# BolinLai/CSTS

Measured on AMD Instinct MI355X. Metric: clips/sec training (fwd+bwd) CSTS-Ego4D 16x256^2 bf16, higher is better.
Workload: dtype bf16; 1 GPU; CSTS_Ego4D_Gaze_Forecast.yaml train step (fwd + KLDiv + 0.05*EgoNCE + bwd + clip + AdamW), 16x256^2 video + 24 kHz STFT audio, b=4/GPU; mode=train, global_batch=4, frames=16, crop=256, parallelism=dp1, step=hip_graph, hip_graph=True, rccl_ranks=1

## Files before the change

csts_amd/csrc/gemm.hip:

```cpp
#include "common.h"
#include "gemm_shared.h"
#include <type_traits>
#include <cstdio>
#include <cstdlib>

namespace {

constexpr int BM = 128, BN = 128, BK = 32, NT_ = 256;
constexpr int KC_LD_BF = BK + 8;
constexpr int OC_LD_BF = 128 + 32;
constexpr int KC_LD_F = BK + 1;
constexpr int OC_LD_F = 128 + 4;

template <bool F32> struct Cmp;
template <> struct Cmp<false> { typedef bf16 T; };
template <> struct Cmp<true> { typedef float T; };


__device__ __forceinline__ void load8(const void* p, int dt, int64_t idx, int nvalid, bool vec, float (&o)[8]) {
  if (nvalid >= 8 && vec) {
    ld8_as_f32(p, dt, idx, o);
  } else {
#pragma unroll
    for (int j = 0; j < 8; ++j) o[j] = (j < nvalid) ? ld_as_f32(p, dt, idx + j) : 0.f;
// ... 1030 lines not shown
bool v3_ok(const csts_gemm_args* a, int split) {
  return v2_ok(a) && a->layout == CSTS_GEMM_NT && a->a_dt == CSTS_BF16 && a->b_dt == CSTS_BF16 && a->K % 16 == 0 &&
         split == 1 && a->colsum == nullptr &&
         a->M * a->lda < (int64_t(1) << 30) && a->N * a->ldb < (int64_t(1) << 30);
}
bool pick3(const csts_gemm_args* a, int split, int* mt, int* stages) {
  if (a->algo != 0 || a->tile_rows != 0 || !v3_ok(a, split) || a->M < 256 || a->res_up[3] > 0) return false;
  if (cdiv(a->M, 128) * cdiv(a->N, BN) >= 512 || a->K < 768) return false;
  *mt = 1;
  *stages = 3;
  return true;
}

bool pick4(const csts_gemm_args* a, int split, int* variant) {
  static const bool enabled = [] { const char* e = getenv("CSTS_GEMM4"); return !(e && e[0] == '0'); }();
  if (!enabled || a->algo != 0 || a->tile_rows != 0 || !v3_ok(a, split) || a->K % 64 != 0 || a->M < 2048 || a->res_up[3] > 0) return false;
  if (a->c_dt == CSTS_F32 && a->residual != nullptr) {
    static const bool res_on = [] { const char* e = getenv("CSTS_GEMM4_RES"); return !(e && e[0] == '0'); }();
    if (!res_on || a->r_dt != CSTS_F32 || a->res_row_mod != 0 || a->epilogue != CSTS_EPI_NONE || a->M % 128 != 0) return false;
    static const bool t64 = [] { const char* e = getenv("CSTS_GEMM4_T64"); return e && (e[0] == '1' || e[0] == '3'); }();
    if (t64 && a->N % 192 == 0 && a->M % 64 == 0 && a->K >= 384 && (a->M / 128) * (a->N / 192) <= 128 && (a->M / 64) * (a->N / 192) >= 64) {
      *variant = 73;
      return true;
    }
    if (a->N % 192 != 0 || (a->M / 128) * (a->N / 192) < 128) return false;
    *variant = 63;
    return true;
  }
  if (a->c_dt != CSTS_BF16 || a->residual != nullptr) return false;
  const int64_t rows = cdiv(a->M, 128);
  {
// ... 12 lines not shown
    return true;
  }
  const int64_t t128 = rows * cdiv(a->N, 128);
  if (a->N % 128 == 0 && t128 >= 128 && t128 <= 512) {
    *variant = a->K >= 1024 ? 33 : 32;
    return true;
  }
  return false;
}

bool pick5(const csts_gemm_args* a, int split) {
  static const bool enabled = [] { const char* e = getenv("CSTS_GEMM5"); return !(e && e[0] == '0'); }();
  if (!enabled || a->algo != 0 || a->tile_rows != 0 || a->M < 16384) return false;
  static const bool k384 = [] { const char* e = getenv("CSTS_GEMM5_K384"); return e && e[0] == '1'; }();
  if (a->K == 384 && !k384) return false;
  return csts_gemm5_ok(a, split);
}

template <int MT>
void launch3_mt(const Params& p, int stages, dim3 grid, hipStream_t s) {
  if (stages == 2) hipLaunchKernelGGL((gemm3_kernel<MT, 2>), grid, dim3(256), 0, s, p);
  else if (stages == 4 && MT < 4) hipLaunchKernelGGL((gemm3_kernel<MT, (MT < 4 ? 4 : 3)>), grid, dim3(256), 0, s, p);
  else hipLaunchKernelGGL((gemm3_kernel<MT, 3>), grid, dim3(256), 0, s, p);
}
void launch3(Params p, int mt, int stages, int wpc, hipStream_t s) {
  const int64_t ntiles = cdiv(p.M, 64 * mt) * p.ntiles_n;
  p.ntiles = ntiles;
  const int stage_bytes = (64 * mt + 128) * 128;
  const int fit = std::max(1, (160 * 1024) / (stages * stage_bytes));
  if (wpc <= 0 || wpc > fit) wpc = fit;
// ... 58 lines not shown
  else hipLaunchKernelGGL((gemm_tiny_kernel<LAYOUT, true>), dim3((unsigned)cdiv(outs, 4)), dim3(256), 0, s, p);
}


enum Family { TINY, GENERIC, V2, RING3, G4, G5 };
struct Route {
  Family family;
  int split;
  bool det;
  int tile_rows, stages;
  int variant, wpc;
  int64_t k_chunk;
  int nsplit;
};

int route(const csts_gemm_args* a, Route* r) {
  *r = Route{};
  r->split = r->nsplit = 1;
  if (tiny_ok(a)) {
    r->family = TINY;
    return 0;
  }
  const int split = r->split = a->split_k > 1 ? a->split_k : 1;
  r->det = split > 1 && a->workspace != nullptr;
  const bool use_v2 = v2_ok(a);
  const int bk = use_v2 ? BK2 : BK;
  r->k_chunk = cdiv(cdiv(a->K, bk), split) * bk;
  r->nsplit = (int)cdiv(a->K, r->k_chunk);
  const int forced = a->algo % 1000;
  if (a->res_up[3] > 0) {
    const int Ti = a->res_up[0], Hi = a->res_up[1], Wi = a->res_up[2], To = a->res_up[3], Ho = a->res_up[4], Wo = a->res_up[5];
    auto p2 = [](int v) { return v > 0 && (v & (v - 1)) == 0; };
    CSTS_REQUIRE(a->residual != nullptr && a->res_row_mod == 0 && split == 1, "res_up needs a residual, no res_row_mod, split_k == 1");
    CSTS_REQUIRE(Ti > 0 && Hi > 0 && Wi > 0 && p2(To) && p2(Ho) && p2(Wo), "res_up: fine grid sizes must be powers of two");
    CSTS_REQUIRE(To >= Ti && Ho >= Hi && Wo >= Wi && a->M % ((int64_t)To * Ho * Wo) == 0, "res_up: M must be B * To * Ho * Wo");
    CSTS_REQUIRE(forced < 300, "res_up is not available in the persistent LDS-DMA kernels");
  }
  if (forced >= 300 && forced < 400) {
    CSTS_REQUIRE(v3_ok(a, split), "algo 3xx (persistent LDS-DMA NT kernel) not applicable to this problem");
    const int code = forced - 300, mt = code / 10, st = code % 10;
    CSTS_REQUIRE((mt == 1 || mt == 2 || mt == 4) && st >= 2 && st <= 4 && !(mt == 4 && st == 4), "bad algo 3xx code");
    r->family = RING3; r->tile_rows = 64 * mt; r->stages = st; r->wpc = a->algo / 1000;
    return 0;
  }
  if (forced >= 400 && forced < 500) {
    CSTS_REQUIRE(v3_ok(a, split), "algo 4xx (8-wave LDS-DMA NT kernel) not applicable to this problem");
    CSTS_REQUIRE(a->K % 64 == 0, "algo 4xx needs K % 64 == 0 (no k-tail instantiations)");
    r->family = G4; r->variant = forced - 400; r->wpc = a->algo / 1000;
    return 0;
  }
  if (forced == 500 || forced == 503 || forced == 506) {
    CSTS_REQUIRE(csts_gemm5_ok(a, split), "algo 500 (streaming thin-operand NT kernel) not applicable to this problem");
    r->family = G5;
    return 0;
  }
  int mt3;
  if (pick5(a, split)) r->family = G5;
  else if (pick4(a, split, &r->variant)) r->family = G4;
  else if (pick3(a, split, &mt3, &r->stages)) { r->family = RING3; r->tile_rows = 64 * mt3; }
  else if (use_v2) { r->family = V2; r->tile_rows = pick_tile_rows(a, cdiv(a->N, BN) * r->nsplit); }
  else { r->family = GENERIC; r->tile_rows = BM; }
  return 0;
}

Params fill_params(const csts_gemm_args* a, const Route& r) {
  Params p{};
// ... 156 lines not shown
```

csts_amd/csrc/gemm4.hip:

```cpp
#include "gemm_shared.h"
#include <algorithm>
#include <cstdio>
#include <type_traits>

#ifdef CSTS_GEMM4_STAMPS
#define G4_STAMP() do { if (stamp_on && nstamp < 500) stamp_buf[nstamp++] = (unsigned long long)__builtin_amdgcn_s_memtime(); } while (0)
#else
#define G4_STAMP() do { } while (0)
#endif

namespace {

template <int WM, int MT, int NT, int S, int NP_ = 0> struct G4 {
  static constexpr int NP = NP_;
  static constexpr int DB = (MT * NT >= 6) ? 1 : 2;
  static constexpr int NWAVES = WM * 2, NTHR = 64 * (NWAVES + NP);
  static constexpr int DW = NP > 0 ? NP : NWAVES;
  static constexpr int BM = WM * 32 * MT, BN = 64 * NT;
  static constexpr int A_BYTES = BM * 128, B_BYTES = BN * 128, STAGE = A_BYTES + B_BYTES;
  static constexpr int NA = BM / 8 / DW, NB = BN / 8 / DW, LPT = NA + NB;
  static constexpr int FIT = (160 * 1024) / (S * STAGE);
  static constexpr int WG = NP > 0 ? 1 : (FIT < 1 ? 1 : (FIT > 2 ? 2 : FIT));
  static constexpr int WPS = (WG * (NWAVES + NP) + 3) / 4;
  static_assert(BM % (8 * DW) == 0 && BN % (8 * DW) == 0, "pieces must divide over the issuing waves");
// ... 108 lines not shown
  int cidx = 0, cstage = 0;

  for (int64_t t = t_first; t < t_end; t += stride) {
    f32x16 acc[MT][NT];
#pragma unroll
    for (int i = 0; i < MT; ++i)
#pragma unroll
      for (int j = 0; j < NT; ++j)
#pragma unroll
        for (int r = 0; r < 16; ++r) acc[i][j][r] = 0.f;
    const int64_t m0 = (t / p.ntiles_n) * BM + wm * 32 * MT + (lane & 31), n0 = (t % p.ntiles_n) * BN + wn * 32 * NT + 4 * hi;

    auto kstep = [&](auto nks_tag, int kt) {
      constexpr int NKS = decltype(nks_tag)::value;
      if constexpr (NP == 0) {
        constexpr int EPI_ST = (FORM == 0 || FORM == 5) ? 0 : MT * NT * 2;
        static_assert(2 * LPT + EPI_ST <= 63, "vmcnt immediate");
        const int ahead = min(S - 2, total_k - 1 - cidx);
        if (EPI_ST > 0 && STORE_AWARE && t != t_first && kt < S - 1) {
          if (S >= 4 && ahead == 2) wait_vm<2 * LPT + EPI_ST>();
          else if (S >= 3 && ahead >= 1) wait_vm<LPT + EPI_ST>();
          else wait_vm<EPI_ST>();
        } else {
          if (S >= 4 && ahead == 2) wait_vm<2 * LPT>();
          else if (S >= 3 && ahead >= 1) wait_vm<LPT>();
          else wait_vm<0>();
        }
      }
      G4_STAMP();
      __builtin_amdgcn_s_barrier();
      G4_STAMP();
// ... 18 lines not shown
      frags(0, 0);
#pragma unroll
      for (int ks = 0; ks < NKS; ++ks) {
        if (DB == 2 && ks + 1 < NKS) frags(ks + 1, (ks + 1) & 1);
        if (refill) {
#pragma unroll
          for (int i = 0; i < LPT; ++i) {
            const bool mine = (NKS == 4) ? (i * 4 / LPT == ks) : (ks == 0);
            if (mine) issue(i, st, k0, full);
          }
        }
#pragma unroll
        for (int i = 0; i < MT; ++i)
#pragma unroll
          for (int j = 0; j < NT; ++j)
            if constexpr (FORM == 5) acc[i][j] = CSTS_MFMA16(fa[ks & (DB - 1)][i], fb[ks & (DB - 1)][j], acc[i][j], 0, 0, 0);
            else acc[i][j] = CSTS_MFMA16(fb[ks & (DB - 1)][j], fa[ks & (DB - 1)][i], acc[i][j], 0, 0, 0);
        if (DB == 1 && ks + 1 < NKS) frags(ks + 1, 0);
      }
      if (refill) advance();
      G4_STAMP();
    };
    for (int kt = 0; kt < nk_full; ++kt) kstep(std::integral_constant<int, 4>(), kt);
    if constexpr (KTAIL) {
      if (k_tail == 1) kstep(std::integral_constant<int, 1>(), nk_full);
      else if (k_tail == 2) kstep(std::integral_constant<int, 2>(), nk_full);
      else if (k_tail == 3) kstep(std::integral_constant<int, 3>(), nk_full);
    }

    G4_STAMP();
    if constexpr (FORM == 5) {
      float* __restrict__ Cf = reinterpret_cast<float*>(p.C);
      const float* __restrict__ Rf = reinterpret_cast<const float*>(p.residual);
      const int64_t mb = m0 - (lane & 31) + 4 * hi, nb = n0 - 4 * hi + (lane & 31);
#pragma unroll
      for (int mi = 0; mi < MT; ++mi) {
        const int64_t mrow = mb + mi * 32;
        float sc[16];
        if (p.row_scale != nullptr) {
          const int64_t s_lo = (mrow - 4 * hi) / p.rows_per_scale, s_hi = (mrow - 4 * hi + 31) / p.rows_per_scale;
          if (s_lo == s_hi) {
            const float v = p.row_scale[s_lo];
#pragma unroll
            for (int r = 0; r < 16; ++r) sc[r] = v;
          } else {
#pragma unroll
            for (int r = 0; r < 16; ++r) sc[r] = p.row_scale[(mrow + (r & 3) + 8 * (r >> 2)) / p.rows_per_scale];
          }
        }
        float rr[2][16];
        const int64_t nwave = n0 - 4 * hi;
        auto loads = [&](int ni, int buf) {
          if (nwave + ni * 32 >= p.N) return;
#pragma unroll
          for (int r = 0; r < 16; ++r) rr[buf][r] = Rf[(mrow + (r & 3) + 8 * (r >> 2)) * p.ldr + nb + ni * 32];
        };
        loads(0, 0);
#pragma unroll
        for (int ni = 0; ni < NT; ++ni) {
          const int cur = ni & 1;
          if (nwave + ni * 32 >= p.N) break;
          const float bq = p.bias != nullptr ? p.bias[nb + ni * 32] : 0.f;
          if (ni + 1 < NT) loads(ni + 1, cur ^ 1);
#pragma unroll
          for (int r = 0; r < 16; ++r) {
            float v = acc[mi][ni][r] + bq;
            if (p.row_scale != nullptr) v *= sc[r];
            Cf[(mrow + (r & 3) + 8 * (r >> 2)) * p.ldc + nb + ni * 32] = v + rr[cur][r];
          }
          __builtin_amdgcn_sched_barrier(0);
        }
      }
    } else if constexpr (FORM != 0) {
      bf16* __restrict__ Cb = reinterpret_cast<bf16*>(p.C);
      bf16* __restrict__ Xb = reinterpret_cast<bf16*>(p.aux);
      const int hi16 = hi << 4;
      auto fwd = [&](auto gelu_tag) {
        constexpr bool GELU = decltype(gelu_tag)::value;
        const float* __restrict__ bias = p.bias;
#pragma unroll
        for (int mi = 0; mi < MT; ++mi) {
          const int64_t m = m0 + mi * 32;
          float bu[NT];
#pragma unroll
          for (int ni = 0; ni < NT; ++ni) bu[ni] = bias[n0 - 4 * hi + ni * 32 + (lane & 31)];
// ... 105 lines not shown
        }
        st4x4(p.C, p.c_dt, m * p.ldc + n0 + ni * 32, o, mok, n0 + ni * 32, p.N, hi);
      }
    }
    }
    G4_STAMP();
  }
  wait_vm<0>();
  G4_STAMP();
#ifdef CSTS_GEMM4_STAMPS
  if (stamp_on) { stamp_buf[0] = (unsigned long long)nstamp; stamp_buf[501] = (unsigned long long)__builtin_amdgcn_s_memrealtime(); }
#endif
}

int gemm4_form(const Params& p, int BM, int BN) {
  if (p.M % BM == 0 && p.N % 32 == 0 && p.c_dt == CSTS_F32 && p.residual != nullptr && p.r_dt == CSTS_F32 && p.res_row_mod == 0 && p.ru_To == 0 &&
      p.epilogue == CSTS_EPI_NONE && p.split_k <= 1)
    return 5;
  if (p.M % BM != 0 || p.N % BN != 0 || p.c_dt != CSTS_BF16 || p.residual != nullptr || p.row_scale != nullptr) return 0;
  if (p.bias != nullptr) {
    if (p.epilogue == CSTS_EPI_NONE) return 1;
    if (p.epilogue == CSTS_EPI_GELU && (p.aux == nullptr || p.aux_dt == CSTS_BF16)) return 2;
    return 0;
  }
  if (p.epilogue == CSTS_EPI_NONE) return 3;
  if (p.epilogue == CSTS_EPI_DGELU && p.aux != nullptr && p.aux_dt == CSTS_BF16) return 4;
  return 0;
}

template <int WM, int MT, int NT, int S, bool FORMS, int NP>
void launch4(Params p, int form, int wpc, hipStream_t s) {
  typedef G4<WM, MT, NT, S, NP> G;
  const int64_t ntiles = cdiv(p.M, G::BM) * cdiv(p.N, G::BN);
  p.ntiles = ntiles;
  p.ntiles_n = (int)cdiv(p.N, G::BN);
  if (wpc <= 0 || wpc > G::WG) wpc = G::WG;
  const int64_t g = std::min<int64_t>(cdiv(ntiles, 8) * 8, (int64_t)256 * wpc);
  const dim3 grid((unsigned)g), block(G::NTHR);
  if constexpr (FORMS) {
    if (form == 1) { hipLaunchKernelGGL((gemm4_kernel<WM, MT, NT, S, 1, NP>), grid, block, 0, s, p); return; }
    if (form == 2) { hipLaunchKernelGGL((gemm4_kernel<WM, MT, NT, S, 2, NP>), grid, block, 0, s, p); return; }
    if (form == 3) { hipLaunchKernelGGL((gemm4_kernel<WM, MT, NT, S, 3, NP>), grid, block, 0, s, p); return; }
    if (form == 4) { hipLaunchKernelGGL((gemm4_kernel<WM, MT, NT, S, 4, NP>), grid, block, 0, s, p); return; }
    if (form == 5) { hipLaunchKernelGGL((gemm4_kernel<WM, MT, NT, S, 5, NP>), grid, block, 0, s, p); return; }
  }
  hipLaunchKernelGGL((gemm4_kernel<WM, MT, NT, S, 0, NP>), grid, block, 0, s, p);
}

#define G4_VARIANTS(X) \
  X(2, 4, 2, 2, 2, false, 0) X(3, 4, 2, 2, 3, false, 0) X(12, 4, 2, 3, 2, false, 0) X(22, 4, 2, 4, 2, false, 0) \
  X(32, 4, 1, 2, 2, true, 0) X(33, 4, 1, 2, 3, true, 0) X(34, 4, 1, 2, 4, true, 0) X(62, 4, 1, 3, 2, true, 0) X(63, 4, 1, 3, 3, true, 0) \
  X(64, 4, 1, 3, 4, true, 0) X(42, 4, 1, 4, 2, false, 0) X(52, 2, 2, 2, 2, false, 0) X(72, 2, 1, 3, 2, true, 0) X(73, 2, 1, 3, 3, true, 0) \
  X(74, 2, 1, 3, 4, true, 0) X(83, 4, 1, 3, 3, true, 4) X(84, 4, 1, 2, 3, true, 4)

struct Variant {
  int code, wm, mt, nt, s, np;
  bool forms;
  void (*launch)(Params, int form, int wpc, hipStream_t);
};
#define X(code, wm, mt, nt, st, forms, np) {code, wm, mt, nt, st, np, forms, launch4<wm, mt, nt, st, forms, np>},
const Variant VARIANTS[] = {G4_VARIANTS(X)};
#undef X

const Variant* resolve4(const Params& p, int variant, int* form) {
  if (p.K % BK2 != 0) return nullptr;
  for (const Variant& v : VARIANTS)
    if (v.code == variant) {
      *form = v.forms ? gemm4_form(p, v.wm * 32 * v.mt, 64 * v.nt) : 0;
      return &v;
    }
  return nullptr;
}

}

bool csts_gemm4_launch(const csts_gemm_params& p, int variant, int wpc, hipStream_t s) {
  int form;
  const Variant* v = resolve4(p, variant, &form);
  if (v != nullptr) v->launch(p, form, wpc, s);
  return v != nullptr;
}

bool csts_gemm4_name(const csts_gemm_params& p, int variant, char* buf, int buflen) {
// ... 6 lines not shown
```

csts_amd/csrc/gemm5.hip:

```cpp
#include "gemm_shared.h"
#include <algorithm>
#include <cstdio>
#include <cstdlib>

namespace {

template <int KCH, int NB, int W> struct G5 {
  static constexpr int K = 96 * KCH, NW = 32 * NB, NTHR = 64 * W;
  static constexpr int CHUNK = 32 * 192;
  static constexpr int RING = 2 * CHUNK;
  static constexpr int BL = 2 * K + 16;
  static constexpr int B_BYTES = NW * BL, A_BYTES = W * RING, LDS = B_BYTES + A_BYTES;
  static constexpr int NPAIR = NB / 2, NSINGLE = NB % 2;
  static constexpr int NDMA = 6 * KCH;
  static_assert(LDS <= 160 * 1024, "weights + rings exceed the CU's LDS");
  static_assert((BL / 16) % 2 == 1, "weight row stride must be an odd number of 16-byte groups");
};

template <int N> struct MinC { static constexpr int v = N < 63 ? N : 63; };

template <int KCH, int NB, int W, int FORM>
__global__ __launch_bounds__((G5<KCH, NB, W>::NTHR), 2) void gemm5_kernel(Params p, int nt_n, int units) {
  typedef G5<KCH, NB, W> G;
  constexpr int K = G::K, BL = G::BL, CHUNK = G::CHUNK, NPAIR = G::NPAIR, NSINGLE = G::NSINGLE, NDMA = G::NDMA;
  constexpr bool C32 = FORM >= 3, RES = FORM == 3, GELU = FORM == 1, DGELU = FORM == 2;
  static_assert(KCH == 1 || KCH == 2 || (KCH == 4 && !DGELU), "K = 96, 192, or 384 without the x gelu' form");
  __shared__ __attribute__((aligned(1024))) char smem[G::LDS];
  const int tid = threadIdx.x, lane = tid & 63, r32 = lane & 31, hi = lane >> 5;
  const int wave = __builtin_amdgcn_readfirstlane(tid >> 6);
  char* const Bs = smem;
  char* const As = smem + G::B_BYTES + wave * G::RING;

  const int grp = blockIdx.x >> 3, ntile = grp % nt_n;
  const int wg = (grp / nt_n) * 8 + (blockIdx.x & 7), nwg = gridDim.x / nt_n;
  const int gw = wg * W + wave, nw = nwg * W;
  const int64_t n0 = (int64_t)ntile * G::NW;

  {
    constexpr int CPR = K / 8;
    const bf16* __restrict__ Bg = reinterpret_cast<const bf16*>(p.B);
// ... 43 lines not shown

  int u = gw;
  if (u < units) {
#pragma unroll
    for (int j = 0; j < (KCH < 2 ? KCH : 2); ++j) issue_chunk(u, 0, j);
  }
  __syncthreads();

  constexpr int NRL = (RES || DGELU) ? 16 * (NPAIR + NSINGLE) : 0;
  constexpr int NST = 16 * (NPAIR + NSINGLE);
  float2 rp[RES ? 16 : 1][NPAIR > 0 ? NPAIR : 1], rp_n[RES ? 16 : 1][NPAIR > 0 ? NPAIR : 1];
  float rs1[RES && NSINGLE ? 16 : 1], rs1_n[RES && NSINGLE ? 16 : 1];
  bf16x2 hp[DGELU ? 16 : 1][NPAIR > 0 ? NPAIR : 1], hp_n[DGELU ? 16 : 1][NPAIR > 0 ? NPAIR : 1];
  bf16 hs1[DGELU && NSINGLE ? 16 : 1], hs1_n[DGELU && NSINGLE ? 16 : 1];
  float rsc = 1.f, rsc_n = 1.f;
  auto request = [&](int un) {
    const int64_t mn = (int64_t)un * 32;
    if constexpr (RES) {
      const float* __restrict__ res = reinterpret_cast<const float*>(p.residual) + (mn + 4 * hi) * p.ldr + n0;
#pragma unroll
      for (int r = 0; r < 16; ++r) {
        const float* row = res + ((r & 3) + 8 * (r >> 2)) * p.ldr;
#pragma unroll
        for (int j = 0; j < NPAIR; ++j) rp_n[r][j] = *reinterpret_cast<const float2*>(row + 64 * j + 2 * r32);
        if constexpr (NSINGLE) rs1_n[r] = row[64 * NPAIR + r32];
      }
      if (p.row_scale != nullptr) rsc_n = p.row_scale[mn / p.rows_per_scale];
    }
    if constexpr (DGELU) {
      const bf16* __restrict__ hx = reinterpret_cast<const bf16*>(p.aux) + (mn + 4 * hi) * p.ldaux + n0;
#pragma unroll
      for (int r = 0; r < 16; ++r) {
        const bf16* row = hx + ((r & 3) + 8 * (r >> 2)) * p.ldaux;
#pragma unroll
        for (int j = 0; j < NPAIR; ++j) hp_n[r][j] = *reinterpret_cast<const bf16x2*>(row + 64 * j + 2 * r32);
        if constexpr (NSINGLE) hs1_n[r] = row[64 * NPAIR + r32];
      }
    }
  };
  constexpr bool AHEAD = RES;
  if (AHEAD && u < units) request(u);

  for (int it = 0; u < units; u += nw, ++it) {
    const int64_t m0 = (int64_t)u * 32;
    if constexpr (NRL > 0 && !AHEAD) {
      request(u);
      wait_vm<MinC<NRL>::v>();
    } else if constexpr (KCH <= 2) {
      if (it == 0) wait_vm<0>();
      else wait_vm<MinC<NST>::v>();
    }
    if constexpr (AHEAD && KCH <= 2) {
#pragma unroll
      for (int r = 0; r < 16; ++r) {
#pragma unroll
        for (int j = 0; j < NPAIR; ++j) {
          if constexpr (RES) rp[r][j] = rp_n[r][j];
          if constexpr (DGELU) hp[r][j] = hp_n[r][j];
        }
        if constexpr (RES && NSINGLE) rs1[r] = rs1_n[r];
        if constexpr (DGELU && NSINGLE) hs1[r] = hs1_n[r];
      }
// ... 37 lines not shown
      if (it == 0) { if (more) wait_vm<24>(); else wait_vm<12>(); }
      else { if (more) wait_vm<MinC<24 + NST>::v>(); else wait_vm<MinC<12 + NST>::v>(); }
#pragma unroll
      for (int r = 0; r < 16; ++r) {
#pragma unroll
        for (int j = 0; j < NPAIR; ++j) rp[r][j] = rp_n[r][j];
        if constexpr (NSINGLE) rs1[r] = rs1_n[r];
      }
      rsc = rsc_n;
    }
    if (AHEAD && more) request(u + nw);
    if constexpr (NRL > 0 && !AHEAD) {
      if (more) wait_vm<MinC<NDMA>::v>();
      else wait_vm<0>();
    }

    if constexpr (C32) {
      float* __restrict__ Cf = reinterpret_cast<float*>(p.C) + (m0 + 4 * hi) * p.ldc + n0;
#pragma unroll
      for (int r = 0; r < 16; ++r) {
        float* row = Cf + ((r & 3) + 8 * (r >> 2)) * p.ldc;
#pragma unroll
        for (int j = 0; j < NPAIR; ++j) {
          float v0 = acc[2 * j][r] + bias_p[j][0], v1 = acc[2 * j + 1][r] + bias_p[j][1];
          if constexpr (RES) {
            if (p.row_scale != nullptr) { v0 *= rsc; v1 *= rsc; }
            v0 += rp[r][j].x; v1 += rp[r][j].y;
          }
          *reinterpret_cast<float2*>(row + 64 * j + 2 * r32) = make_float2(v0, v1);
        }
        if constexpr (NSINGLE) {
          float v = acc[NB - 1][r] + bias_s;
          if constexpr (RES) {
            if (p.row_scale != nullptr) v *= rsc;
            v += rs1[r];
          }
          row[64 * NPAIR + r32] = v;
        }
      }
    } else {
      bf16* __restrict__ Cb = reinterpret_cast<bf16*>(p.C) + (m0 + 4 * hi) * p.ldc + n0;
      bf16* __restrict__ Hb = GELU && p.aux != nullptr ? reinterpret_cast<bf16*>(p.aux) + (m0 + 4 * hi) * p.ldaux + n0 : nullptr;
#pragma unroll
      for (int r = 0; r < 16; ++r) {
        const int ro = (r & 3) + 8 * (r >> 2);
#pragma unroll
// ... 15 lines not shown
          if constexpr (GELU) {
            if (Hb != nullptr) Hb[ro * p.ldaux + 64 * NPAIR + r32] = (bf16)v;
            v = gelu_fast(v);
          }
          if constexpr (DGELU) v *= dgelu_fast((float)hs1_n[r]);
          Cb[ro * p.ldc + 64 * NPAIR + r32] = (bf16)v;
        }
      }
    }
  }
  wait_vm<0>();
}

int gemm5_form(const csts_gemm_args* a) {
  if (a->residual != nullptr) {
    if (a->c_dt == CSTS_F32 && a->r_dt == CSTS_F32 && a->res_row_mod == 0 && a->res_up[3] == 0 && a->epilogue == CSTS_EPI_NONE &&
        (a->row_scale == nullptr || (a->rows_per_scale > 0 && a->rows_per_scale % 32 == 0)))
      return 3;
    return -1;
  }
  if (a->row_scale != nullptr) return -1;
  if (a->c_dt == CSTS_F32) return a->epilogue == CSTS_EPI_NONE ? 4 : -1;
  if (a->c_dt != CSTS_BF16) return -1;
  if (a->epilogue == CSTS_EPI_NONE) return 0;
  if (a->epilogue == CSTS_EPI_GELU && a->aux_dt == CSTS_BF16) return 1;
  if (a->epilogue == CSTS_EPI_DGELU && a->aux != nullptr && a->aux_dt == CSTS_BF16) return 2;
  return -1;
}

template <int KCH, int NB, int W = 8>
bool launch5(const Params& p, int form, hipStream_t s) {
  typedef G5<KCH, NB, W> G;
  const int nt_n = (int)(p.N / G::NW), units = (int)(p.M / 32);
  const int g = (256 / (8 * nt_n)) * 8 * nt_n;
  const dim3 grid((unsigned)g), block(G::NTHR);
  switch (form) {
    case 0: hipLaunchKernelGGL((gemm5_kernel<KCH, NB, W, 0>), grid, block, 0, s, p, nt_n, units); return true;
    case 1: hipLaunchKernelGGL((gemm5_kernel<KCH, NB, W, 1>), grid, block, 0, s, p, nt_n, units); return true;
    case 2:
      if constexpr (KCH != 4) { hipLaunchKernelGGL((gemm5_kernel<KCH, NB, W, 2>), grid, block, 0, s, p, nt_n, units); return true; }
      return false;
    case 3:
      if constexpr (NB == 3) { hipLaunchKernelGGL((gemm5_kernel<KCH, NB, W, 3>), grid, block, 0, s, p, nt_n, units); return true; }
      return false;
    case 4: hipLaunchKernelGGL((gemm5_kernel<KCH, NB, W, 4>), grid, block, 0, s, p, nt_n, units); return true;
  }
  return false;
}

int gemm5_nb(const csts_gemm_args* a) {
  static const int wide192 = [] { const char* e = getenv("CSTS_GEMM5_WIDE192"); return e ? atoi(e) : 0; }();
  if (gemm5_form(a) == 3) return 3;
  if (a->K == 96) return a->N % 192 == 0 ? 6 : 3;
  if (a->K == 384) return 3;
  return (a->N % 192 == 0 && (a->algo % 1000 == 506 || (a->algo % 1000 != 503 && wide192))) ? 6 : 3;
}

}

bool csts_gemm5_ok(const csts_gemm_args* a, int split) {
  if (a->layout != CSTS_GEMM_NT || a->compute != CSTS_BF16 || a->a_dt != CSTS_BF16 || a->b_dt != CSTS_BF16 || split != 1) return false;
  if (a->colsum != nullptr || (a->K != 96 && a->K != 192 && a->K != 384) || a->N % 96 != 0 || a->N > 768 || a->M % 32 != 0 || a->M < 32) return false;
  if (gemm5_form(a) < 0) return false;
  if (a->K == 384 && (gemm5_form(a) == 2 || a->N > 384)) return false;
  auto al = [](const void* q) { return (reinterpret_cast<uintptr_t>(q) & 15) == 0; };
  if (!al(a->A) || !al(a->B) || !al(a->C) || a->lda % 8 != 0 || a->ldb % 8 != 0 || a->ldc % 2 != 0) return false;
  if (a->aux != nullptr && (!al(a->aux) || a->ldaux % 2 != 0)) return false;
// ... 26 lines not shown
```

csts_amd/csrc/gemm_shared.h:

```cpp
#pragma once
#include "common.h"

struct csts_gemm_params {
  const void* A; const void* B; void* C;
  const float* bias; void* aux; const void* residual; const float* row_scale; float* ws;
  float* colsum; float* colsum_ws;
  int64_t lda, ldb, ldc, ldaux, ldr;
  int64_t M, N, K, res_row_mod, rows_per_scale, k_chunk;
  int a_dt, b_dt, c_dt, aux_dt, r_dt, epilogue, split_k, a_vec, b_vec, ntiles_n;
  int64_t ntiles;
  unsigned long long* stamps;
  int res_lines;
  int store_aware;
  int ru_Ti, ru_Hi, ru_Wi, ru_To, ru_Ho, ru_Wo, ru_lw, ru_lh, ru_lt;
};

namespace {

constexpr int BK2 = 64;

typedef csts_gemm_params Params;

template <int N> __device__ __forceinline__ void wait_vm() { asm volatile("s_waitcnt vmcnt(%0)" ::"n"(N) : "memory"); }

// ... 83 lines not shown
        const int64_t at = (r.base + (int64_t)(r.ti[a] * p.ru_Hi + r.hi[e]) * p.ru_Wi + r.wi[f]) * p.ldr + n;
        if constexpr (NV == 8) {
          float v[8];
          ld8_as_f32(p.residual, p.r_dt, at, v);
#pragma unroll
          for (int j = 0; j < 8; ++j) acc[j] += wgt * v[j];
        } else {
#pragma unroll
          for (int j = 0; j < NV; ++j) acc[j] += wgt * ld_as_f32(p.residual, p.r_dt, at + j);
        }
      }
    }
  }
}

__device__ __forceinline__ void st4x4_bf16_whole(bf16* base, int64_t at, const f32x4 (&o)[4], int hi) {
  uint2 pk[4];
#pragma unroll
  for (int q = 0; q < 4; ++q) {
    const bf16x4 b = {(bf16)o[q][0], (bf16)o[q][1], (bf16)o[q][2], (bf16)o[q][3]};
    pk[q] = __builtin_bit_cast(uint2, b);
  }
#pragma unroll
  for (int pr = 0; pr < 2; ++pr) {
    uint2 a = pk[2 * pr], b = pk[2 * pr + 1];
    const auto rx = __builtin_amdgcn_permlane32_swap(a.x, b.x, false, false);
    const auto ry = __builtin_amdgcn_permlane32_swap(a.y, b.y, false, false);
    a.x = rx[0]; b.x = rx[1]; a.y = ry[0]; b.y = ry[1];
    *reinterpret_cast<uint4*>(base + at - 4 * hi + 16 * pr + 8 * hi) = make_uint4(a.x, a.y, b.x, b.y);
  }
// ... 21 lines not shown
```

Before: 209.4 clips/s.

## Fuse trilinear upsampled-skip residual into gemm4/gemm5 LDS-DMA epilogues

Adds new epilogue forms to the 8-wave gemm4 kernel and the streaming gemm5 kernel. These forms read a coarse residual and trilinearly upsample it into the output, with specialised integer-weight fast paths for 2x spatial and 2x temporal upsampling. Before this, any GEMM with res_up set was excluded from these faster kernels and routed to the older generic/v2 path. The change lets the large multiscale skip-connection GEMMs use the faster kernels. In exchange it adds more template instantiations and gathered loads in the epilogue that are not coalesced, and it raises register pressure.

Result: no change. 210.4 clips/s (median of 6 runs) (+0.5%).

```diff
diff --git a/csts_amd/csrc/gemm.hip b/csts_amd/csrc/gemm.hip
--- a/csts_amd/csrc/gemm.hip
+++ b/csts_amd/csrc/gemm.hip
@@ -1068,7 +1068,13 @@
 
 bool pick4(const csts_gemm_args* a, int split, int* variant) {
   static const bool enabled = [] { const char* e = getenv("CSTS_GEMM4"); return !(e && e[0] == '0'); }();
-  if (!enabled || a->algo != 0 || a->tile_rows != 0 || !v3_ok(a, split) || a->K % 64 != 0 || a->M < 2048 || a->res_up[3] > 0) return false;
+  if (!enabled || a->algo != 0 || a->tile_rows != 0 || !v3_ok(a, split) || a->K % 64 != 0 || a->M < 2048) return false;
+  if (a->res_up[3] > 0) {
+    const int64_t coarse_rows = a->M / ((int64_t)a->res_up[3] * a->res_up[4] * a->res_up[5]) * a->res_up[0] * a->res_up[1] * a->res_up[2];
+    if (a->c_dt != CSTS_F32 || a->residual == nullptr || coarse_rows * a->ldr >= (int64_t(1) << 30)) return false;
+    if (res_up_mode(a->res_up[0], a->res_up[1], a->res_up[2], a->res_up[3], a->res_up[4], a->res_up[5], a->M, a->ldr) == 3) return false;
+    if (a->N % 192 != 0 || (a->M / 128) * (a->N / 192) < 512) return false;
+  }
   if (a->c_dt == CSTS_F32 && a->residual != nullptr) {
     static const bool res_on = [] { const char* e = getenv("CSTS_GEMM4_RES"); return !(e && e[0] == '0'); }();
     if (!res_on || a->r_dt != CSTS_F32 || a->res_row_mod != 0 || a->epilogue != CSTS_EPI_NONE || a->M % 128 != 0) return false;
@@ -1111,6 +1117,7 @@
   if (!enabled || a->algo != 0 || a->tile_rows != 0 || a->M < 16384) return false;
   static const bool k384 = [] { const char* e = getenv("CSTS_GEMM5_K384"); return e && e[0] == '1'; }();
   if (a->K == 384 && !k384) return false;
+  if (a->res_up[3] > 0 && res_up_mode(a->res_up[0], a->res_up[1], a->res_up[2], a->res_up[3], a->res_up[4], a->res_up[5], a->M, a->ldr) != 2) return false;
   return csts_gemm5_ok(a, split);
 }
 
@@ -1199,6 +1206,8 @@
   int nsplit;
 };
 
+Params fill_params(const csts_gemm_args* a, const struct Route& r);
+
 int route(const csts_gemm_args* a, Route* r) {
   *r = Route{};
   r->split = r->nsplit = 1;
@@ -1219,7 +1228,19 @@
     CSTS_REQUIRE(a->residual != nullptr && a->res_row_mod == 0 && split == 1, "res_up needs a residual, no res_row_mod, split_k == 1");
     CSTS_REQUIRE(Ti > 0 && Hi > 0 && Wi > 0 && p2(To) && p2(Ho) && p2(Wo), "res_up: fine grid sizes must be powers of two");
     CSTS_REQUIRE(To >= Ti && Ho >= Hi && Wo >= Wi && a->M % ((int64_t)To * Ho * Wo) == 0, "res_up: M must be B * To * Ho * Wo");
-    CSTS_REQUIRE(forced < 300, "res_up is not available in the persistent LDS-DMA kernels");
+    const int mode = res_up_mode(Ti, Hi, Wi, To, Ho, Wo, a->M, a->ldr);
+    bool carried = forced < 300;
+    if (forced == 468 || forced == 478 || ((forced == 463 || forced == 473) && mode != 3)) {
+      char name[96];
+      const bool eight = forced % 10 == 8;
+      carried = v3_ok(a, split) && a->K % 64 == 0 && (!eight || mode == 3) &&
+                csts_gemm4_name(fill_params(a, *r), forced - 400 - (eight ? 5 : 0), name, (int)sizeof(name));
+    } else if (forced == 500 || forced == 503 || forced == 506) {
+      carried = mode == 2 && csts_gemm5_ok(a, split);
+    } else if (forced == 508) {
+      carried = mode != 2 && csts_gemm5_ok(a, split);
+    }
+    if (!carried) CSTS_REQUIRE(forced < 300, "res_up is not available in the persistent LDS-DMA kernels");
   }
   if (forced >= 300 && forced < 400) {
     CSTS_REQUIRE(v3_ok(a, split), "algo 3xx (persistent LDS-DMA NT kernel) not applicable to this problem");
@@ -1232,9 +1253,10 @@
     CSTS_REQUIRE(v3_ok(a, split), "algo 4xx (8-wave LDS-DMA NT kernel) not applicable to this problem");
     CSTS_REQUIRE(a->K % 64 == 0, "algo 4xx needs K % 64 == 0 (no k-tail instantiations)");
     r->family = G4; r->variant = forced - 400; r->wpc = a->algo / 1000;
+    if (a->res_up[3] > 0 && forced % 10 == 8) r->variant -= 5;
     return 0;
   }
-  if (forced == 500 || forced == 503 || forced == 506) {
+  if (forced == 500 || forced == 503 || forced == 506 || (forced == 508 && a->res_up[3] > 0)) {
     CSTS_REQUIRE(csts_gemm5_ok(a, split), "algo 500 (streaming thin-operand NT kernel) not applicable to this problem");
     r->family = G5;
     return 0;
diff --git a/csts_amd/csrc/gemm4.hip b/csts_amd/csrc/gemm4.hip
--- a/csts_amd/csrc/gemm4.hip
+++ b/csts_amd/csrc/gemm4.hip
@@ -146,7 +146,7 @@
     auto kstep = [&](auto nks_tag, int kt) {
       constexpr int NKS = decltype(nks_tag)::value;
       if constexpr (NP == 0) {
-        constexpr int EPI_ST = (FORM == 0 || FORM == 5) ? 0 : MT * NT * 2;
+        constexpr int EPI_ST = (FORM == 0 || FORM >= 5) ? 0 : MT * NT * 2;
         static_assert(2 * LPT + EPI_ST <= 63, "vmcnt immediate");
         const int ahead = min(S - 2, total_k - 1 - cidx);
         if (EPI_ST > 0 && STORE_AWARE && t != t_first && kt < S - 1) {
@@ -195,7 +195,7 @@
         for (int i = 0; i < MT; ++i)
 #pragma unroll
           for (int j = 0; j < NT; ++j)
-            if constexpr (FORM == 5) acc[i][j] = CSTS_MFMA16(fa[ks & (DB - 1)][i], fb[ks & (DB - 1)][j], acc[i][j], 0, 0, 0);
+            if constexpr (FORM >= 5) acc[i][j] = CSTS_MFMA16(fa[ks & (DB - 1)][i], fb[ks & (DB - 1)][j], acc[i][j], 0, 0, 0);
             else acc[i][j] = CSTS_MFMA16(fb[ks & (DB - 1)][j], fa[ks & (DB - 1)][i], acc[i][j], 0, 0, 0);
         if (DB == 1 && ks + 1 < NKS) frags(ks + 1, 0);
       }
@@ -210,13 +210,94 @@
     }
 
     G4_STAMP();
-    if constexpr (FORM == 5) {
+    if constexpr (FORM >= 5) {
+      constexpr int RU = FORM - 5;
       float* __restrict__ Cf = reinterpret_cast<float*>(p.C);
       const float* __restrict__ Rf = reinterpret_cast<const float*>(p.residual);
       const int64_t mb = m0 - (lane & 31) + 4 * hi, nb = n0 - 4 * hi + (lane & 31);
 #pragma unroll
       for (int mi = 0; mi < MT; ++mi) {
         const int64_t mrow = mb + mi * 32;
+        const int64_t nwave = n0 - 4 * hi;
+        if constexpr (RU != 0) {
+          float sc1 = 1.f;
+          bool sc_uni = true;
+          if (p.row_scale != nullptr) {
+            const int64_t s_lo = (mrow - 4 * hi) / p.rows_per_scale, s_hi = (mrow - 4 * hi + 31) / p.rows_per_scale;
+            sc_uni = s_lo == s_hi;
+            sc1 = p.row_scale[s_lo];
+          }
+          auto finish = [&](int ni, const float (&up)[16], float bq) {
+            if (sc_uni) {
+#pragma unroll
+              for (int r = 0; r < 16; ++r) acc[mi][ni][r] = (acc[mi][ni][r] + bq) * sc1 + up[r];
+            } else {
+#pragma unroll
+              for (int r = 0; r < 16; ++r)
+                acc[mi][ni][r] = (acc[mi][ni][r] + bq) * p.row_scale[(mrow + (r & 3) + 8 * (r >> 2)) / p.rows_per_scale] + up[r];
+            }
+          };
+          auto stores = [&](int ni) {
+#pragma unroll
+            for (int r = 0; r < 16; ++r) Cf[(mrow + (r & 3) + 8 * (r >> 2)) * p.ldc + nb + ni * 32] = acc[mi][ni][r];
+          };
+          if constexpr (RU == 3) {
+#pragma unroll
+            for (int ni = 0; ni < NT; ++ni) {
+              if (nwave + ni * 32 >= p.N) break;
+              const float bq = p.bias != nullptr ? p.bias[nb + ni * 32] : 0.f;
+              int64_t mr = mrow;
+              asm volatile("" : "+v"(mr));
+              float up[16];
+#pragma unroll
+              for (int r = 0; r < 16; ++r) {
+                float u1[1];
+                res_up_load<1>(p, res_up_row(p, mr + (r & 3) + 8 * (r >> 2)), nb + ni * 32, u1);
+                up[r] = u1[0];
+              }
+              finish(ni, up, bq);
+              __builtin_amdgcn_sched_barrier(0);
+              stores(ni);
+              __builtin_amdgcn_sched_barrier(0);
+            }
+          } else {
+            float raw[4][8];
+            const int64_t ncol0 = (t % p.ntiles_n) * BN + wn * 32 * NT;
+            const int lane4 = (lane & 31) * 4;
+            auto taps = [&](int ni) {
+              const char* __restrict__ Rc = reinterpret_cast<const char*>(Rf + ncol0 + ni * 32);
+              int mq = (int)mrow;
+              asm volatile("" : "+v"(mq));
+#pragma unroll
+              for (int q = 0; q < 4; ++q) {
+                int off[8];
+                res_up_quad_offsets<RU>(p, mq + 8 * q, off);
+#pragma unroll
+                for (int k = 0; k < 8; ++k) raw[q][k] = *reinterpret_cast<const float*>(Rc + (unsigned)(off[k] * 4 + lane4));
+              }
+            };
+            taps(0);
+#pragma unroll
+            for (int ni = 0; ni < NT; ++ni) {
+              const float bq = p.bias != nullptr ? p.bias[nb + ni * 32] : 0.f;
+              int mq = (int)mrow;
+              asm volatile("" : "+v"(mq));
+              float up[16];
+#pragma unroll
+              for (int q = 0; q < 4; ++q) {
+                float u4[4];
+                res_up_quad_combine<RU>(p, mq + 8 * q, raw[q], u4);
+#pragma unroll
+                for (int j = 0; j < 4; ++j) up[4 * q + j] = u4[j];
+              }
+              finish(ni, up, bq);
+              __builtin_amdgcn_sched_barrier(0);
+              if (ni + 1 < NT) taps(ni + 1);
+              stores(ni);
+              __builtin_amdgcn_sched_barrier(0);
+            }
+          }
+        } else {
         float sc[16];
         if (p.row_scale != nullptr) {
           const int64_t s_lo = (mrow - 4 * hi) / p.rows_per_scale, s_hi = (mrow - 4 * hi + 31) / p.rows_per_scale;
@@ -230,7 +311,6 @@
           }
         }
         float rr[2][16];
-        const int64_t nwave = n0 - 4 * hi;
         auto loads = [&](int ni, int buf) {
           if (nwave + ni * 32 >= p.N) return;
 #pragma unroll
@@ -250,6 +330,7 @@
             Cf[(mrow + (r & 3) + 8 * (r >> 2)) * p.ldc + nb + ni * 32] = v + rr[cur][r];
           }
           __builtin_amdgcn_sched_barrier(0);
+        }
         }
       }
     } else if constexpr (FORM != 0) {
@@ -385,9 +466,12 @@
 }
 
 int gemm4_form(const Params& p, int BM, int BN) {
-  if (p.M % BM == 0 && p.N % 32 == 0 && p.c_dt == CSTS_F32 && p.residual != nullptr && p.r_dt == CSTS_F32 && p.res_row_mod == 0 && p.ru_To == 0 &&
-      p.epilogue == CSTS_EPI_NONE && p.split_k <= 1)
-    return 5;
+  if (p.M % BM == 0 && p.N % 32 == 0 && p.c_dt == CSTS_F32 && p.residual != nullptr && p.r_dt == CSTS_F32 && p.res_row_mod == 0 &&
+      p.epilogue == CSTS_EPI_NONE && p.split_k <= 1) {
+    if (p.ru_To == 0) return 5;
+    const int64_t coarse_rows = p.M / ((int64_t)p.ru_To * p.ru_Ho * p.ru_Wo) * p.ru_Ti * p.ru_Hi * p.ru_Wi;
+    if (coarse_rows * p.ldr < (int64_t(1) << 30) && p.N % BN == 0) return 5 + res_up_mode(p.ru_Ti, p.ru_Hi, p.ru_Wi, p.ru_To, p.ru_Ho, p.ru_Wo, p.M, p.ldr);
+  }
   if (p.M % BM != 0 || p.N % BN != 0 || p.c_dt != CSTS_BF16 || p.residual != nullptr || p.row_scale != nullptr) return 0;
   if (p.bias != nullptr) {
     if (p.epilogue == CSTS_EPI_NONE) return 1;
@@ -398,6 +482,8 @@
   if (p.epilogue == CSTS_EPI_DGELU && p.aux != nullptr && p.aux_dt == CSTS_BF16) return 4;
   return 0;
 }
+
+#define G4_RES_UP(MT, NT, S, NP) ((MT) == 1 && (NT) == 3 && (S) == 3 && (NP) == 0)
 
 template <int WM, int MT, int NT, int S, bool FORMS, int NP>
 void launch4(Params p, int form, int wpc, hipStream_t s) {
@@ -414,6 +500,11 @@
     if (form == 3) { hipLaunchKernelGGL((gemm4_kernel<WM, MT, NT, S, 3, NP>), grid, block, 0, s, p); return; }
     if (form == 4) { hipLaunchKernelGGL((gemm4_kernel<WM, MT, NT, S, 4, NP>), grid, block, 0, s, p); return; }
     if (form == 5) { hipLaunchKernelGGL((gemm4_kernel<WM, MT, NT, S, 5, NP>), grid, block, 0, s, p); return; }
+    if constexpr (G4_RES_UP(MT, NT, S, NP)) {
+      if (form == 6) { hipLaunchKernelGGL((gemm4_kernel<WM, MT, NT, S, 6, NP>), grid, block, 0, s, p); return; }
+      if (form == 7) { hipLaunchKernelGGL((gemm4_kernel<WM, MT, NT, S, 7, NP>), grid, block, 0, s, p); return; }
+      if (form == 8) { hipLaunchKernelGGL((gemm4_kernel<WM, MT, NT, S, 8, NP>), grid, block, 0, s, p); return; }
+    }
   }
   hipLaunchKernelGGL((gemm4_kernel<WM, MT, NT, S, 0, NP>), grid, block, 0, s, p);
 }
@@ -438,6 +529,7 @@
   for (const Variant& v : VARIANTS)
     if (v.code == variant) {
       *form = v.forms ? gemm4_form(p, v.wm * 32 * v.mt, 64 * v.nt) : 0;
+      if (p.ru_To > 0 && !(*form > 5 && G4_RES_UP(v.mt, v.nt, v.s, v.np))) return nullptr;
       return &v;
     }
   return nullptr;
diff --git a/csts_amd/csrc/gemm5.hip b/csts_amd/csrc/gemm5.hip
--- a/csts_amd/csrc/gemm5.hip
+++ b/csts_amd/csrc/gemm5.hip
@@ -23,7 +23,9 @@
 __global__ __launch_bounds__((G5<KCH, NB, W>::NTHR), 2) void gemm5_kernel(Params p, int nt_n, int units) {
   typedef G5<KCH, NB, W> G;
   constexpr int K = G::K, BL = G::BL, CHUNK = G::CHUNK, NPAIR = G::NPAIR, NSINGLE = G::NSINGLE, NDMA = G::NDMA;
-  constexpr bool C32 = FORM >= 3, RES = FORM == 3, GELU = FORM == 1, DGELU = FORM == 2;
+  constexpr bool C32 = FORM >= 3, RES = FORM == 3 || FORM >= 5, GELU = FORM == 1, DGELU = FORM == 2;
+  constexpr bool RU2 = FORM == 5, RUG = FORM == 6;
+  static_assert(FORM < 5 || (KCH == 2 && NB == 3), "the up-sampled-skip forms: K = 192 on 96-column tiles");
   static_assert(KCH == 1 || KCH == 2 || (KCH == 4 && !DGELU), "K = 96, 192, or 384 without the x gelu' form");
   __shared__ __attribute__((aligned(1024))) char smem[G::LDS];
   const int tid = threadIdx.x, lane = tid & 63, r32 = lane & 31, hi = lane >> 5;
@@ -97,9 +99,36 @@
   bf16x2 hp[DGELU ? 16 : 1][NPAIR > 0 ? NPAIR : 1], hp_n[DGELU ? 16 : 1][NPAIR > 0 ? NPAIR : 1];
   bf16 hs1[DGELU && NSINGLE ? 16 : 1], hs1_n[DGELU && NSINGLE ? 16 : 1];
   float rsc = 1.f, rsc_n = 1.f;
+  float2 tp_n[RU2 ? 4 : 1][RU2 ? 8 : 1];
+  float ts_n[RU2 ? 4 : 1][RU2 ? 8 : 1];
   auto request = [&](int un) {
     const int64_t mn = (int64_t)un * 32;
-    if constexpr (RES) {
+    if constexpr (RU2) {
+      const char* __restrict__ resb = reinterpret_cast<const char*>(reinterpret_cast<const float*>(p.residual) + n0);
+#pragma unroll
+      for (int q = 0; q < 4; ++q) {
+        int off[8];
+        res_up_quad_offsets<2>(p, (int)mn + 4 * hi + 8 * q, off);
+#pragma unroll
+        for (int k = 0; k < 8; ++k) {
+          tp_n[q][k] = *reinterpret_cast<const float2*>(resb + (unsigned)(off[k] * 4 + 8 * r32));
+          if (q == 3 && k == 7) wait_vm<63>();
+          ts_n[q][k] = *reinterpret_cast<const float*>(resb + 256 + (unsigned)(off[k] * 4 + 4 * r32));
+        }
+      }
+      if (p.row_scale != nullptr) rsc = p.row_scale[mn / p.rows_per_scale];
+    } else if constexpr (RUG) {
+#pragma unroll
+      for (int r = 0; r < 16; ++r) {
+        const ResUpRow rw = res_up_row(p, mn + 4 * hi + (r & 3) + 8 * (r >> 2));
+        float up2[2], up1[1];
+        res_up_load<2>(p, rw, n0 + 2 * r32, up2);
+        res_up_load<1>(p, rw, n0 + 64 + r32, up1);
+        rp[r][0] = make_float2(up2[0], up2[1]);
+        rs1[r] = up1[0];
+      }
+      if (p.row_scale != nullptr) rsc = p.row_scale[mn / p.rows_per_scale];
+    } else if constexpr (RES) {
       const float* __restrict__ res = reinterpret_cast<const float*>(p.residual) + (mn + 4 * hi) * p.ldr + n0;
 #pragma unroll
       for (int r = 0; r < 16; ++r) {
@@ -121,14 +150,14 @@
       }
     }
   };
-  constexpr bool AHEAD = RES;
+  constexpr bool AHEAD = RES && !RUG && !RU2;
   if (AHEAD && u < units) request(u);
 
   for (int it = 0; u < units; u += nw, ++it) {
     const int64_t m0 = (int64_t)u * 32;
     if constexpr (NRL > 0 && !AHEAD) {
       request(u);
-      wait_vm<MinC<NRL>::v>();
+      if constexpr (!RU2) wait_vm<RUG ? 0 : MinC<NRL>::v>();
     } else if constexpr (KCH <= 2) {
       if (it == 0) wait_vm<0>();
       else wait_vm<MinC<NST>::v>();
@@ -196,6 +225,25 @@
       if (more) wait_vm<MinC<NDMA>::v>();
       else wait_vm<0>();
     }
+    if constexpr (RU2) {
+#pragma unroll
+      for (int q = 0; q < 4; ++q) {
+        float vx[8], vy[8], vs[8], ox[4], oy[4], os[4];
+#pragma unroll
+        for (int k = 0; k < 8; ++k) { vx[k] = tp_n[q][k].x; vy[k] = tp_n[q][k].y; vs[k] = ts_n[q][k]; }
+        res_up_quad_combine<2>(p, (int)m0 + 4 * hi + 8 * q, vx, ox);
+        res_up_quad_combine<2>(p, (int)m0 + 4 * hi + 8 * q, vy, oy);
+        res_up_quad_combine<2>(p, (int)m0 + 4 * hi + 8 * q, vs, os);
+#pragma unroll
+        for (int j = 0; j < 4; ++j) {
+          const int r = 4 * q + j;
+          float v0 = acc[0][r] + bias_p[0][0], v1 = acc[1][r] + bias_p[0][1], v = acc[2][r] + bias_s;
+          if (p.row_scale != nullptr) { v0 *= rsc; v1 *= rsc; v *= rsc; }
+          acc[0][r] = v0 + ox[j]; acc[1][r] = v1 + oy[j]; acc[2][r] = v + os[j];
+        }
+      }
+      __builtin_amdgcn_sched_barrier(0);
+    }
 
     if constexpr (C32) {
       float* __restrict__ Cf = reinterpret_cast<float*>(p.C) + (m0 + 4 * hi) * p.ldc + n0;
@@ -204,6 +252,7 @@
         float* row = Cf + ((r & 3) + 8 * (r >> 2)) * p.ldc;
 #pragma unroll
         for (int j = 0; j < NPAIR; ++j) {
+          if constexpr (RU2) { *reinterpret_cast<float2*>(row + 64 * j + 2 * r32) = make_float2(acc[2 * j][r], acc[2 * j + 1][r]); continue; }
           float v0 = acc[2 * j][r] + bias_p[j][0], v1 = acc[2 * j + 1][r] + bias_p[j][1];
           if constexpr (RES) {
             if (p.row_scale != nullptr) { v0 *= rsc; v1 *= rsc; }
@@ -212,6 +261,7 @@
           *reinterpret_cast<float2*>(row + 64 * j + 2 * r32) = make_float2(v0, v1);
         }
         if constexpr (NSINGLE) {
+          if constexpr (RU2) { row[64 * NPAIR + r32] = acc[NB - 1][r]; continue; }
           float v = acc[NB - 1][r] + bias_s;
           if constexpr (RES) {
             if (p.row_scale != nullptr) v *= rsc;
@@ -257,9 +307,14 @@
 
 int gemm5_form(const csts_gemm_args* a) {
   if (a->residual != nullptr) {
-    if (a->c_dt == CSTS_F32 && a->r_dt == CSTS_F32 && a->res_row_mod == 0 && a->res_up[3] == 0 && a->epilogue == CSTS_EPI_NONE &&
-        (a->row_scale == nullptr || (a->rows_per_scale > 0 && a->rows_per_scale % 32 == 0)))
-      return 3;
+    if (a->c_dt == CSTS_F32 && a->r_dt == CSTS_F32 && a->res_row_mod == 0 && a->epilogue == CSTS_EPI_NONE &&
+        (a->row_scale == nullptr || (a->rows_per_scale > 0 && a->rows_per_scale % 32 == 0))) {
+      if (a->res_up[3] == 0) return 3;
+      const int Ti = a->res_up[0], Hi = a->res_up[1], Wi = a->res_up[2], To = a->res_up[3], Ho = a->res_up[4], Wo = a->res_up[5];
+      const int64_t coarse_rows = a->M / ((int64_t)To * Ho * Wo) * Ti * Hi * Wi;
+      if (a->K != 192 || coarse_rows * a->ldr >= (int64_t(1) << 30)) return -1;
+      return res_up_mode(Ti, Hi, Wi, To, Ho, Wo, a->M, a->ldr) == 2 ? 5 : 6;
+    }
     return -1;
   }
   if (a->row_scale != nullptr) return -1;
@@ -286,6 +341,12 @@
     case 3:
       if constexpr (NB == 3) { hipLaunchKernelGGL((gemm5_kernel<KCH, NB, W, 3>), grid, block, 0, s, p, nt_n, units); return true; }
       return false;
+    case 5:
+      if constexpr (NB == 3 && KCH == 2) { hipLaunchKernelGGL((gemm5_kernel<KCH, NB, W, 5>), grid, block, 0, s, p, nt_n, units); return true; }
+      return false;
+    case 6:
+      if constexpr (NB == 3 && KCH == 2) { hipLaunchKernelGGL((gemm5_kernel<KCH, NB, W, 6>), grid, block, 0, s, p, nt_n, units); return true; }
+      return false;
     case 4: hipLaunchKernelGGL((gemm5_kernel<KCH, NB, W, 4>), grid, block, 0, s, p, nt_n, units); return true;
   }
   return false;
@@ -293,7 +354,7 @@
 
 int gemm5_nb(const csts_gemm_args* a) {
   static const int wide192 = [] { const char* e = getenv("CSTS_GEMM5_WIDE192"); return e ? atoi(e) : 0; }();
-  if (gemm5_form(a) == 3) return 3;
+  if (gemm5_form(a) == 3 || gemm5_form(a) >= 5) return 3;
   if (a->K == 96) return a->N % 192 == 0 ? 6 : 3;
   if (a->K == 384) return 3;
   return (a->N % 192 == 0 && (a->algo % 1000 == 506 || (a->algo % 1000 != 503 && wide192))) ? 6 : 3;
diff --git a/csts_amd/csrc/gemm_shared.h b/csts_amd/csrc/gemm_shared.h
--- a/csts_amd/csrc/gemm_shared.h
+++ b/csts_amd/csrc/gemm_shared.h
@@ -121,6 +121,88 @@
   }
 }
 
+template <int R>
+__device__ __forceinline__ void res_up_axis_int(int o, int in, int& i0, int& i1, float& l0, float& l1) {
+  if constexpr (R == 1) {
+    i0 = o; i1 = o; l1 = 0.f; l0 = 1.f;
+  } else {
+    i0 = o > 0 ? (o - 1) >> 1 : 0;
+    i1 = i0 + (i0 < in - 1 ? 1 : 0);
+    l1 = o == 0 ? 0.f : ((o & 1) ? 0.25f : 0.75f);
+    l0 = 1.f - l1;
+  }
+}
+template <int RT, int RH, int RW>
+__device__ __forceinline__ float res_up_combine(const ResUpRow& r, const float (&v)[RT * RH * RW]) {
+  float acc = 0.f;
+#pragma unroll
+  for (int k = 0; k < RT * RH * RW; ++k) {
+    const int a = RT == 2 ? k / (RH * RW) : 0, e = RH == 2 ? (k / RW) % RH : 0, f = RW == 2 ? k % RW : 0;
+    const float wgt = r.tl[a] * r.hl[e] * r.wl[f];
+    const bool skip = (a == 1 && r.tl[1] == 0.f) || (e == 1 && r.hl[1] == 0.f) || (f == 1 && r.wl[1] == 0.f);
+    acc = skip ? acc : acc + wgt * v[k];
+  }
+  return acc;
+}
+template <int RU>
+__device__ __forceinline__ void res_up_quad_offsets(const Params& p, int m4, int (&off)[8]) {
+  const int ls = p.ru_lw + p.ru_lh, ld = (int)p.ldr;
+  if constexpr (RU == 1) {
+    const int ow4 = m4 & (p.ru_Wo - 1), oh = (m4 >> p.ru_lw) & (p.ru_Ho - 1), tb = m4 >> ls;
+    int h[2];
+    float l0, l1;
+    res_up_axis_int<2>(oh, p.ru_Hi, h[0], h[1], l0, l1);
+    const int k2 = ow4 >> 1, line = __mul24(p.ru_Wi, ld);
+    const int c1 = __mul24(k2, ld), c0 = k2 > 0 ? c1 - ld : c1, c2 = c1 + ld, c3 = k2 + 2 < p.ru_Wi ? c2 + ld : c2;
+    const int r0 = __mul24(__mul24(tb, p.ru_Hi) + h[0], line), r1 = h[1] != h[0] ? r0 + line : r0;
+    off[0] = r0 + c0; off[1] = r0 + c1; off[2] = r0 + c2; off[3] = r0 + c3;
+    off[4] = r1 + c0; off[5] = r1 + c1; off[6] = r1 + c2; off[7] = r1 + c3;
+  } else {
+    const int sp4 = m4 & ((1 << ls) - 1), ot = (m4 >> ls) & (p.ru_To - 1), b = m4 >> (ls + p.ru_lt);
+    int t[2];
+    float l0, l1;
+    res_up_axis_int<2>(ot, p.ru_Ti, t[0], t[1], l0, l1);
+    const int f0 = __mul24(((__mul24(b, p.ru_Ti) + t[0]) << ls) + sp4, ld), f1 = t[1] != t[0] ? f0 + (ld << ls) : f0;
+#pragma unroll
+    for (int j = 0; j < 4; ++j) { off[j] = f0 + j * ld; off[4 + j] = f1 + j * ld; }
+  }
+}
+template <int RU>
+__device__ __forceinline__ void res_up_quad_combine(const Params& p, int m4, const float (&v)[8], float (&out)[4]) {
+  const int ls = p.ru_lw + p.ru_lh;
+  ResUpRow r;
+  int i0, i1;
+  if constexpr (RU == 1) {
+    const int ow4 = m4 & (p.ru_Wo - 1), oh = (m4 >> p.ru_lw) & (p.ru_Ho - 1);
+    r.tl[0] = 1.f; r.tl[1] = 0.f;
+    res_up_axis_int<2>(oh, p.ru_Hi, i0, i1, r.hl[0], r.hl[1]);
+#pragma unroll
+    for (int j = 0; j < 4; ++j) {
+      if (j == 0) res_up_axis_int<2>(ow4, p.ru_Wi, i0, i1, r.wl[0], r.wl[1]);
+      else { r.wl[1] = (j & 1) ? 0.25f : 0.75f; r.wl[0] = 1.f - r.wl[1]; }
+      const int c = j == 0 ? 0 : (j == 3 ? 2 : 1);
+      const float vv[4] = {v[c], v[c + 1], v[4 + c], v[4 + c + 1]};
+      out[j] = res_up_combine<1, 2, 2>(r, vv);
+    }
+  } else {
+    const int ot = (m4 >> ls) & (p.ru_To - 1);
+    res_up_axis_int<2>(ot, p.ru_Ti, i0, i1, r.tl[0], r.tl[1]);
+    r.hl[0] = 1.f; r.hl[1] = 0.f; r.wl[0] = 1.f; r.wl[1] = 0.f;
+#pragma unroll
+    for (int j = 0; j < 4; ++j) {
+      const float vv[2] = {v[j], v[4 + j]};
+      out[j] = res_up_combine<2, 1, 1>(r, vv);
+    }
+  }
+}
+__host__ inline int res_up_mode(int Ti, int Hi, int Wi, int To, int Ho, int Wo, int64_t M, int64_t ldr) {
+  const int64_t coarse_rows = M / ((int64_t)To * Ho * Wo) * Ti * Hi * Wi;
+  if (Wo % 4 != 0 || M >= (int64_t(1) << 31) || coarse_rows >= (1 << 24) || Wi * ldr >= (1 << 24)) return 3;
+  if (To == Ti && Ho == 2 * Hi && Wo == 2 * Wi) return 1;
+  if (To == 2 * Ti && Ho == Hi && Wo == Wi) return 2;
+  return 3;
+}
+
 __device__ __forceinline__ void st4x4_bf16_whole(bf16* base, int64_t at, const f32x4 (&o)[4], int hi) {
   uint2 pk[4];
 #pragma unroll
```
